# kdexd/probnmn-clevr

Hardware: AMD Instinct MI355X
Metric: CLEVR questions/sec (joint_training step) (higher is better)
Workload: dtype f32; 1 GPU; joint_training_ours.yml (NMN + seq2seq + REINFORCE), global batch 1024 = 1024 questions per GPU x 1 (BASELINE configs[3]), 14x14x1024 features, half of the batch with program supervision, fwd+bwd+[all-reduce]+clamp+Adam; global_batch=1024, per_gpu_batch=1024, parallelism=dp1

## Files before the change

### probnmn-clevr_amd/csrc/conv_stream.h

```cpp
#pragma once
#include <hip/hip_runtime.h>
#include <stdint.h>

#include <type_traits>

#include "../../include/probnmn_hip.h"
#include "global_ptr.h"

#ifdef PNMN_STREAM_CYCLES
#define PNMN_CYC() __builtin_readcyclecounter()
#else
#define PNMN_CYC() 0ull
#endif

namespace pnmn {
namespace stream {

constexpr int CB = 128;
constexpr int QC = 32;
constexpr int NTHREADS = 512;
constexpr int LOADER_WAVE = 4;
constexpr int NLOAD = 4;
constexpr int MTILES = 13;
constexpr int TAB_ROWS = 208;

using lchar = __attribute__((address_space(3))) char;

template <int H, int W, int TH>
struct Geom {
    static constexpr bool WHOLE = (TH == H);
    static constexpr int NB = H / TH;
    static constexpr int RP = (WHOLE ? H : TH + 2) * W;
    static constexpr int Z0 = (RP + 7) & ~7;
    static constexpr int SUB_PIECES = (Z0 + 15) / 16;
    static constexpr int PIECES = 2 * SUB_PIECES;
    static constexpr int SUB_BYTES = (Z0 + 8) * 64;
    static constexpr int SLOT_BYTES = 2 * SUB_BYTES;
    static constexpr int RING = WHOLE ? 6 : 4;
    static constexpr bool OVERLAP = (Z0 % 16) != 0;
    static constexpr int owner(int i) { return (OVERLAP && i == SUB_PIECES - 1) ? (SUB_PIECES - 2) % NLOAD : i % NLOAD; }
    static constexpr int owned(int lw) {
        int n = 0;
        for (int i = 0; i < SUB_PIECES; ++i) n += owner(i) == lw ? 1 : 0;
        return n;
    }
    static constexpr int TAB_OFF = RING * SLOT_BYTES;
    static constexpr int LDS_BYTES = TAB_OFF + 9 * TAB_ROWS * 2 + 128;
    static_assert(LDS_BYTES <= 160 * 1024, "ring + table must fit the CU's LDS");
    static_assert((Z0 + 7) * 64 + 16 < 65536 && SUB_BYTES < 65536, "table entries and the kb offset are 16 bits");
};

struct Launch {
    int n_seg;
    int wg_begin[3], split[3], unit0[3], n_units[3], per_xcd[3];
    int wgs_x;
    int total;
    int cin_chunks, ntaps, in_stride, out_stride, relu;
    unsigned long long* dbg;
};

__device__ __forceinline__ void lds_barrier() {
    asm volatile("s_waitcnt lgkmcnt(0)\n\ts_barrier" ::: "memory");
}

template <int H, int W, int TH>
__device__ __forceinline__ bool pass_rows(int band, int dil, int npass, int pass, int ntaps, int& rs, int& re, int& t0, int& t1) {
    if (Geom<H, W, TH>::WHOLE) {
        rs = 0, re = H, t0 = 0, t1 = ntaps;
        return true;
    }
    const int y0 = band * TH;
    if (npass == 1) {
        const int halo = (ntaps == 1) ? 0 : 1;
        rs = y0 - halo < 0 ? 0 : y0 - halo;
        re = y0 + TH + halo > H ? H : y0 + TH + halo;
        t0 = 0, t1 = ntaps;
        return true;
    }
    const int a = y0 + (pass - 1) * dil;
    rs = a < 0 ? 0 : (a > H ? H : a);
    re = a + TH < 0 ? 0 : (a + TH > H ? H : a + TH);
    t0 = 3 * pass, t1 = t0 + 3;
    return re > rs;
}

template <int H, int W, int TH>
struct Walker {
    using G = Geom<H, W, TH>;
    const pnmn_conv_item* items;
    int vid, total;
    int item, band, sub, split, cb;
    int dil, npass, slots;
    int chunk, pass, kq;
    int rs, re, t0, t1;

    __device__ __forceinline__ bool valid() const { return vid < total; }

    __device__ __forceinline__ bool decode(const Launch& L) {
        const int cout_blocks = L.total / L.wgs_x;
        const int s8 = vid >> 3;
        const int cbi = s8 % cout_blocks;
        const int x = (s8 / cout_blocks) * 8 + (vid & 7);
        int wb = L.wg_begin[0], sp = L.split[0], u0 = L.unit0[0], nu = L.n_units[0], per = L.per_xcd[0];
        if (L.n_seg > 1 && x >= L.wg_begin[1]) wb = L.wg_begin[1], sp = L.split[1], u0 = L.unit0[1], nu = L.n_units[1], per = L.per_xcd[1];
        if (L.n_seg > 2 && x >= L.wg_begin[2]) wb = L.wg_begin[2], sp = L.split[2], u0 = L.unit0[2], nu = L.n_units[2], per = L.per_xcd[2];
        const int local = x - wb;
        const int slot = local >> 3;
        const int j = slot / sp;
        const int unit = (local & 7) * per + j;
        if (unit >= nu || j >= per) return false;
        const int u = u0 + unit;
        item = u / G::NB, band = u % G::NB, sub = slot - j * sp, split = sp, cb = cbi;
        return true;
    }
    __device__ __forceinline__ void open_unit(const Launch& L) {
        while (vid < total && !decode(L)) vid += (int)gridDim.x;
        if (vid >= total) return;
        const pnmn_conv_item* it = items + item;
        dil = it->dilation;
        slots = it->gate ? 2 : 1;
        npass = (G::WHOLE || L.ntaps == 1 || dil == 1) ? 1 : 3;
        chunk = 0, pass = 0, kq = 0;
        while (!pass_rows<H, W, TH>(band, dil, npass, pass, L.ntaps, rs, re, t0, t1)) ++pass;
    }
    __device__ __forceinline__ void start(const Launch& L, const pnmn_conv_item* its) {
        items = its, vid = (int)blockIdx.x, total = L.total;
        open_unit(L);
    }
    __device__ __forceinline__ bool next_stage(const Launch& L) {
        if (++kq < 4) return true;
        kq = 0;
        while (++pass < npass)
            if (pass_rows<H, W, TH>(band, dil, npass, pass, L.ntaps, rs, re, t0, t1)) return true;
        if (++chunk >= L.cin_chunks) return false;
        pass = 0;
        while (!pass_rows<H, W, TH>(band, dil, npass, pass, L.ntaps, rs, re, t0, t1)) ++pass;
        return true;
    }
    __device__ __forceinline__ void next_unit(const Launch& L) {
        vid += (int)gridDim.x;
        open_unit(L);
    }
    __device__ __forceinline__ int cbase() const { return chunk * CB + kq * QC; }
};


template <int N>
__device__ __forceinline__ void wait_vm() {
    asm volatile("s_waitcnt vmcnt(%0)" ::"n"(N) : "memory");
}

template <int H, int W, int TH, int LW>
__device__ __forceinline__ void issue_rows(const float* src, int in_stride, int rs, int re, lchar* slot, int lane) {
    using G = Geom<H, W, TH>;
    const int nr = (re - rs) * W;
    using gchar = __attribute__((address_space(1))) char;
    const uint64_t src64 = (uint64_t)(uintptr_t)src + (uint64_t)rs * W * in_stride * 4;
    const uint64_t base64 = ((uint64_t)(uint32_t)__builtin_amdgcn_readfirstlane((int)(src64 >> 32)) << 32) |
                            (uint32_t)__builtin_amdgcn_readfirstlane((int)(uint32_t)src64);
    const gchar* base = (const gchar*)base64;
    const int s = lane & 3, lrow = lane >> 2;
    const int g = (((s & 1) ^ ((lane >> 4) & 1)) << 1) | (s >> 1);
    const uint32_t voff = (uint32_t)(lrow * in_stride + g * 4) * 4u;
    const int edge = (nr & 15) && nr < G::Z0 ? (nr < G::Z0 - 16 ? nr & ~15 : G::Z0 - 16) : -1;
    const uint32_t eoff = edge < 0 ? voff : (uint32_t)(((edge + lrow < nr ? edge + lrow : nr - 1) - edge) * in_stride + g * 4) * 4u;
#pragma unroll
    for (int i = 0; i < G::SUB_PIECES; ++i) {
        if (G::owner(i) != LW) continue;
        const int r0 = i * 16 < G::Z0 - 16 ? i * 16 : G::Z0 - 16;
        const uint32_t off = r0 == edge ? eoff : voff;
        const gchar* pb = base + (size_t)(r0 < nr ? r0 : 0) * in_stride * 4;
        __builtin_amdgcn_global_load_lds((const gfloat*)(pb + off), slot + r0 * 64, 16, 0, 0);
        __builtin_amdgcn_global_load_lds((const gfloat*)(pb + (off + 64u)), slot + G::SUB_BYTES + r0 * 64, 16, 0, 0);
    }
}

template <int H, int W, int TH, int LW>
__device__ __forceinline__ void fixup(char* lds, int slot_x, int slot_g, const float* mask, int rs, int re, bool gated, int lane) {
    using G = Geom<H, W, TH>;
    const int nr = (re - rs) * W;
    const gfloat* msrc = mask ? as_global(mask) + rs * W : nullptr;
    float mk[G::SUB_PIECES];
#pragma unroll
    for (int i = 0; i < G::SUB_PIECES; ++i) {
        if (G::owner(i) != LW) continue;
        const int row = i * 16 + (lane >> 2);
        mk[i] = msrc ? msrc[row < nr ? row : nr - 1] : 1.f;
    }
#pragma unroll
    for (int kb = 0; kb < 2; ++kb) {
        f32x4 v[G::SUB_PIECES], gt[G::SUB_PIECES];
#pragma unroll
        for (int i = 0; i < G::SUB_PIECES; ++i) {
            if (G::owner(i) != LW) continue;
            const int off = kb * G::SUB_BYTES + i * 1024 + lane * 16;
            v[i] = *reinterpret_cast<const f32x4*>(lds + slot_x + off);
            if (gated) gt[i] = *reinterpret_cast<const f32x4*>(lds + slot_g + off);
        }
#pragma unroll
        for (int i = 0; i < G::SUB_PIECES; ++i) {
            if (G::owner(i) != LW) continue;
            const int off = kb * G::SUB_BYTES + i * 1024 + lane * 16;
            f32x4 x = v[i] * mk[i];
            if (gated) {
                x.x = gt[i].x > 0.f ? x.x : 0.f;
                x.y = gt[i].y > 0.f ? x.y : 0.f;
                x.z = gt[i].z > 0.f ? x.z : 0.f;
                x.w = gt[i].w > 0.f ? x.w : 0.f;
            }
            if (i * 16 + (lane >> 2) < G::Z0) *reinterpret_cast<f32x4*>(lds + slot_x + off) = x;
        }
    }
}

template <int H, int W, int TH>
__device__ __forceinline__ void fill_table(char* lds, int band, int dil, int npass, int ntaps, int lane, int w, int nw) {
    using G = Geom<H, W, TH>;
    constexpr int HW = TH * W;
    uint16_t* tab = reinterpret_cast<uint16_t*>(lds + G::TAB_OFF);
    const int y0 = G::WHOLE ? 0 : band * TH;
    const int ntile = ntaps * MTILES;
    for (int t4 = 4 * w; t4 < ntile; t4 += 4 * nw) {
        const int tile = t4 + (lane >> 4);
        const int tap = tile / MTILES;
        const int m = tile - tap * MTILES;
        const int p = m * 16 + (lane & 15);
        int rs, re, t0, t1;
        const int pass = npass == 1 ? 0 : tap / 3;
        const bool rows_ok = tile < ntile && pass_rows<H, W, TH>(band, dil, npass, pass, ntaps, rs, re, t0, t1);
        int dy = 0, dx = 0;
        if (ntaps == 9) dy = (tap / 3 - 1) * dil, dx = (tap % 3 - 1) * dil;
        const int yy = y0 + p / W + dy, xx = p % W + dx;
        const bool ok = rows_ok && p < HW && yy >= rs && yy < re && (unsigned)xx < (unsigned)W;
        const int qv = rows_ok ? (yy - rs) * W + xx : p;
        const int row = ok ? qv : G::Z0 + (qv & 7);
        if (tile < ntile) tab[tap * TAB_ROWS + p] = (uint16_t)(row * 64 + ((row >> 2) & 1) * 16);
    }
}

template <int H, int W, int TH>
__device__ __forceinline__ void start_up(char* lds, const Walker<H, W, TH>& first, int ntaps, int wave, int lane) {
    using G = Geom<H, W, TH>;
    for (int t = wave * 64 + lane; t < G::RING * 64; t += NTHREADS) {
        const int sl = t >> 6, kb = (t >> 5) & 1;
        *reinterpret_cast<f32x4*>(lds + sl * G::SLOT_BYTES + kb * G::SUB_BYTES + G::Z0 * 64 + (t & 31) * 16) = f32x4{0.f, 0.f, 0.f, 0.f};
    }
    if (first.valid()) fill_table<H, W, TH>(lds, first.band, first.dil, first.npass, ntaps, lane, wave, NTHREADS / 64);
    lds_barrier();
}

template <int H, int W, int TH, int LW>
__device__ __forceinline__ void loader(const Launch& L, const pnmn_conv_item* items, char* lds, int lane) {
    using G = Geom<H, W, TH>;
    constexpr int NP2 = 2 * G::owned(LW);
    lchar* ring = (lchar*)lds;
    __builtin_amdgcn_s_setprio(3);
    Walker<H, W, TH> P, C;
    P.start(L, items);
    C = P;
    int issued = 0, freed = 0, cstart = 0;
    const pnmn_conv_item* pit = P.valid() ? items + P.item : nullptr;
    auto top_up = [&](int limit) {
        while (P.valid() && issued - freed + P.slots <= limit) {
            const float* src = (pit->in2 != nullptr && P.chunk > 0) ? pit->in2 + P.kq * QC : pit->in + P.cbase();
            issue_rows<H, W, TH, LW>(src, L.in_stride, P.rs, P.re, ring + (issued % G::RING) * G::SLOT_BYTES, lane);
            if (P.slots == 2) {
                issue_rows<H, W, TH, LW>(pit->gate + P.cbase(), L.in_stride, P.rs, P.re,
                                     ring + ((issued + 1) % G::RING) * G::SLOT_BYTES, lane);
            }
            issued += P.slots;
            if (!P.next_stage(L)) {
                P.next_unit(L);
                pit = P.valid() ? items + P.item : nullptr;
            }
        }
    };
    bool unit_end = false;
    unsigned long long lc[4] = {0, 0, 0, 0};
    unsigned long long lt = PNMN_CYC();
    auto lap = [&](int k) {
        const unsigned long long now = PNMN_CYC();
        lc[k] += now - lt;
        lt = now;
    };
    auto prepare = [&] {
        const pnmn_conv_item* cit = items + C.item;
        const int younger = issued - (cstart + C.slots);
        if (younger == 0) wait_vm<0>();
        else if (younger == 1) wait_vm<NP2>();
        else if (younger == 2) wait_vm<2 * NP2>();
        else wait_vm<3 * NP2>();
        lap(1);
        if (cit->mask != nullptr || C.slots == 2)
            fixup<H, W, TH, LW>(lds, (cstart % G::RING) * G::SLOT_BYTES, ((cstart + 1) % G::RING) * G::SLOT_BYTES, cit->mask, C.rs,
                            C.re, C.slots == 2, lane);
        lap(2);
    };
    top_up(P.valid() ? P.slots : 0);
    int tab_band = C.valid() ? C.band : -1, tab_dil = C.valid() ? C.dil : -1;
    start_up<H, W, TH>(lds, C, L.ntaps, LOADER_WAVE + LW, lane);
    lap(0);
    bool prepared = false;
    while (C.valid()) {
        if (!prepared) prepare();
        if (unit_end) {
            lds_barrier();
            unit_end = false;
            lap(3);
        }
        if (C.band != tab_band || C.dil != tab_dil) {
            fill_table<H, W, TH>(lds, C.band, C.dil, C.npass, L.ntaps, lane, LW, NLOAD);
            tab_band = C.band, tab_dil = C.dil;
        }
        lap(2);
        lds_barrier();
        lap(3);
        freed = cstart;
        cstart += C.slots;
        if (!C.next_stage(L)) {
            C.next_unit(L);
            unit_end = true;
        }
        prepared = C.valid() && issued >= cstart + C.slots;
        if (prepared) prepare();
        top_up(G::RING);
        lap(0);
    }
    if (unit_end) lds_barrier();
    if (L.dbg && lane == 0 && LW == 0) {
        unsigned long long* d = L.dbg + ((size_t)gridDim.x * 4 + blockIdx.x) * 8;
        d[0] = lc[0], d[1] = lc[1], d[2] = lc[2], d[3] = lc[3];
    }
}


__device__ __forceinline__ void mfma(f32x4& acc, float a, float b) {
    asm volatile("v_mfma_f32_16x16x4_f32 %0, %1, %2, %0" : "+v"(acc) : "v"(a), "v"(b));
}


template <int H, int W, int TH, int MTW>
__device__ __forceinline__ void epilogue(const pnmn_conv_item& it, const f32x4* acc, int mbase, int n0, int band, int out_stride,
                                         int relu, int lane, const f32x4 bias4) {
    constexpr int HW = TH * W;
    asm volatile("" : "+v"(lane));
    const int li = lane & 15, g = lane >> 4;
    const int p_img = Geom<H, W, TH>::WHOLE ? 0 : band * TH * W;
    auto act = [&](f32x4 v) {
        v += bias4;
        if (relu) {
            v.x = fmaxf(v.x, 0.f);
            v.y = fmaxf(v.y, 0.f);
            v.z = fmaxf(v.z, 0.f);
            v.w = fmaxf(v.w, 0.f);
        }
        return v;
    };
    float* const out0 = it.out + (size_t)p_img * out_stride + n0 + 4 * g;
    if (!(it.flags & (PNMN_CONV_ACCUMULATE | PNMN_CONV_MASKBWD | PNMN_CONV_DATTN))) {
#pragma unroll
        for (int j = 0; j < MTW; ++j) {
            const int p = (mbase + j) * 16 + li;
            if (p < HW) store4(as_global(out0 + (size_t)p * out_stride), act(acc[j]));
        }
        return;
    }
    if (it.flags & PNMN_CONV_DATTN) {
        const bool dattn = it.mb_attn != nullptr;
        f32x4 fv[MTW];
#pragma unroll
        for (int j = 0; j < MTW; ++j) {
            const int p = (mbase + j) * 16 + li;
            fv[j] = (dattn && p < HW) ? load4(as_global(it.mb_feats) + (size_t)(p_img + p) * CB + n0 + 4 * g) : f32x4{0.f, 0.f, 0.f, 0.f};
        }
#pragma unroll
        for (int j = 0; j < MTW; ++j) {
            const int p = (mbase + j) * 16 + li;
            if (p < HW) store4(as_global(out0 + (size_t)p * out_stride), act(acc[j]));
        }
        if (dattn) {
#pragma unroll
            for (int j = 0; j < MTW; ++j) {
                const int p = (mbase + j) * 16 + li;
                const f32x4 v = acc[j];
                float part = (p < HW) ? v.x * fv[j].x + v.y * fv[j].y + v.z * fv[j].z + v.w * fv[j].w : 0.f;
                part += __shfl_xor(part, 16);
                part += __shfl_xor(part, 32);
                if (p < HW && g == 0) unsafeAtomicAdd(it.mb_dattn + p_img + p, part);
            }
        }
        return;
    }
    if (it.flags & PNMN_CONV_MASKBWD) {
        const bool sole = it.flags & PNMN_CONV_MB_SOLE;
        const gfloat* attn = as_global(it.mb_attn);
        float am[MTW];
        f32x4 fv[MTW], dold[MTW];
#pragma unroll
        for (int j = 0; j < MTW; ++j) {
            const int p = (mbase + j) * 16 + li;
            const bool ok = p < HW;
            am[j] = (ok && attn) ? attn[p_img + p] : 1.f;
            fv[j] = (ok && attn) ? load4(as_global(it.mb_feats) + (size_t)(p_img + p) * CB + n0 + 4 * g) : f32x4{0.f, 0.f, 0.f, 0.f};
            dold[j] = (ok && sole) ? load4(as_global(it.mb_dfeats) + (size_t)(p_img + p) * CB + n0 + 4 * g) : f32x4{0.f, 0.f, 0.f, 0.f};
        }
#pragma unroll
        for (int j = 0; j < MTW; ++j) {
            const int p = (mbase + j) * 16 + li;
            const bool ok = p < HW;
            const f32x4 v = acc[j];
            float part = v.x * fv[j].x + v.y * fv[j].y + v.z * fv[j].z + v.w * fv[j].w;
            if (ok) {
                float* d = it.mb_dfeats + (size_t)(p_img + p) * CB + n0 + 4 * g;
                if (sole) {
                    store4(as_global(d), dold[j] + v * am[j]);
                } else {
                    unsafeAtomicAdd(d + 0, v.x * am[j]);
                    unsafeAtomicAdd(d + 1, v.y * am[j]);
                    unsafeAtomicAdd(d + 2, v.z * am[j]);
                    unsafeAtomicAdd(d + 3, v.w * am[j]);
                }
            }
            if (attn) {
                part += __shfl_xor(part, 16);
                part += __shfl_xor(part, 32);
                if (ok && g == 0) unsafeAtomicAdd(it.mb_dattn + p_img + p, part);
            }
        }
        return;
    }
    if (it.flags & PNMN_CONV_ATOMIC) {
#pragma unroll
        for (int j = 0; j < MTW; ++j) {
            const int p = (mbase + j) * 16 + li;
            if (p < HW) {
                const f32x4 v = act(acc[j]);
                float* d = out0 + (size_t)p * out_stride;
                unsafeAtomicAdd(d + 0, v.x);
                unsafeAtomicAdd(d + 1, v.y);
                unsafeAtomicAdd(d + 2, v.z);
                unsafeAtomicAdd(d + 3, v.w);
            }
        }
        return;
    }
    f32x4 old[MTW];
#pragma unroll
    for (int j = 0; j < MTW; ++j) {
        const int p = (mbase + j) * 16 + li;
        old[j] = p < HW ? load4(as_global(out0 + (size_t)p * out_stride)) : f32x4{0.f, 0.f, 0.f, 0.f};
    }
#pragma unroll
    for (int j = 0; j < MTW; ++j) {
        const int p = (mbase + j) * 16 + li;
        if (p < HW) store4(as_global(out0 + (size_t)p * out_stride), act(acc[j]) + old[j]);
    }
}

template <int H, int W, int TH, int MTW>
__device__ __forceinline__ void epilogue_plain_pair(const pnmn_conv_item& it, const f32x4* acc0, const f32x4* acc1, int mbase, int n0,
                                                    int band, int out_stride, int relu, int lane, const f32x4 bias0, const f32x4 bias1) {
    constexpr int HW = TH * W;
    asm volatile("" : "+v"(lane));
    const int li = lane & 15, g = lane >> 4;
    const int p_img = Geom<H, W, TH>::WHOLE ? 0 : band * TH * W;
    auto act = [&](f32x4 v, const f32x4 b) {
        v += b;
        if (relu) {
            v.x = fmaxf(v.x, 0.f);
            v.y = fmaxf(v.y, 0.f);
            v.z = fmaxf(v.z, 0.f);
            v.w = fmaxf(v.w, 0.f);
        }
        return v;
    };
    float* const out0 = it.out + (size_t)p_img * out_stride + n0 + 4 * g;
#pragma unroll
    for (int j = 0; j < MTW; ++j) {
        const int p = (mbase + j) * 16 + li;
        const f32x4 v0 = act(acc0[j], bias0), v1 = act(acc1[j], bias1);
        if (p < HW) {
            store4(as_global(out0 + (size_t)p * out_stride), v0);
            store4(as_global(out0 + (size_t)p * out_stride + 16), v1);
        }
        __builtin_amdgcn_sched_barrier(0);
    }
}

template <int H, int W, int TH, int SPLIT, int KIND>
__device__ __forceinline__ void run_unit(Walker<H, W, TH>& Wk, const Launch& L, char* lds, int& cstart, int wave, int lane,
                                         unsigned long long (&cyc)[4]) {
    using G = Geom<H, W, TH>;
    using std::integral_constant;
    const unsigned long long c_unit = PNMN_CYC();
    static_assert(SPLIT == 1 || SPLIT == 2 || SPLIT == 4 || SPLIT == 6 || SPLIT == 8 || SPLIT == 14 || SPLIT == 26,
                  "workgroups per 128-channel block");
    constexpr int NW = SPLIT == 1 ? 2 : 1;
    constexpr int MW = SPLIT <= 2 ? 1 : SPLIT / 2;
    constexpr int MTW = (MTILES + MW - 1) / MW;
    constexpr int MH = (MTW + 1) / 2;
    constexpr int WSETS = NW == 2 ? 2 : 3;
    constexpr uint32_t FULL = (1u << MTW) - 1u;
    const int li = lane & 15, g = lane >> 4;
    constexpr bool DEALT = (MW & (MW - 1)) != 0;
    const int gw = Wk.sub * 4 + wave;
    const int nt = DEALT ? 0 : wave % (4 / (DEALT ? 1 : MW));
    const int mbase = DEALT ? (gw % MW) * MTW : (wave / (4 / (DEALT ? 1 : MW))) * MTW;
    const pnmn_conv_item it = Wk.items[Wk.item];
    const int n0 = DEALT ? Wk.cb * CB + (gw / MW) * 16 : Wk.cb * CB + Wk.sub * (CB / SPLIT) + nt * 16 * NW;
    const int band = Wk.band;
    const int cin_total = L.cin_chunks * CB;
    const int slots = Wk.slots;

    f32x4 acc[NW][MTW];
#pragma unroll
    for (int n = 0; n < NW; ++n)
#pragma unroll
        for (int j = 0; j < MTW; ++j) acc[n][j] = f32x4{0.f, 0.f, 0.f, 0.f};

    constexpr int NTAPS = KIND == 2 ? 1 : 9;
    const gfloat* wrow = as_global(it.weight) + (size_t)(n0 + li) * NTAPS * cin_total + 4 * g;
    const size_t wtile = (size_t)16 * NTAPS * cin_total;
    const uint32_t gconst = (uint32_t)((g >> 1) * 16 | (g & 1) * 32);
    uint32_t tab_lane = (uint32_t)(G::TAB_OFF + (mbase * 16 + li) * 2);
    asm volatile("" : "+v"(tab_lane));
    const uint32_t exist = (mbase >= MTILES) ? 0u : (MTILES - mbase >= MTW ? FULL : ((1u << (MTILES - mbase)) - 1u));

    f32x4 bias4[NW];
#pragma unroll
    for (int n = 0; n < NW; ++n) {
        bias4[n] = f32x4{0.f, 0.f, 0.f, 0.f};
        if (it.bias) bias4[n] = load4(as_global(it.bias) + n0 + 16 * n + 4 * g);
    }
    f32x4 wq[WSETS][NW][2];
    auto wload = [&](f32x4 (&dst)[NW][2], const gfloat* p) {
#pragma unroll
        for (int n = 0; n < NW; ++n) {
            dst[n][0] = load4(p + n * wtile);
            dst[n][1] = load4(p + n * wtile + 16);
        }
    };
    {
        const gfloat* w0 = wrow + (size_t)Wk.t0 * cin_total + Wk.cbase();
        wload(wq[0], w0);
        if constexpr (WSETS == 3) wload(wq[1], KIND == 2 ? w0 + QC : w0 + cin_total);
    }

    uint32_t rb[MTW];
    f32x4 afrag[MTW];
    uint32_t slot_base = 0;
    using lf32x4 = __attribute__((address_space(3))) f32x4;
    const uint32_t lds0 = (uint32_t)(uintptr_t)(lchar*)lds;
    auto row_fetch = [&](int j, const char* tp) { rb[j] = *reinterpret_cast<const uint16_t*>(tp + j * 32); };
    auto row_apply = [&](int j) { rb[j] = (rb[j] ^ gconst) + slot_base; };
    auto frag_load = [&](int j, int kb) { afrag[j] = *reinterpret_cast<const lf32x4*>((uintptr_t)(rb[j] + kb * G::SUB_BYTES)); };

    auto half = [&](auto DO, auto LO, auto HI, const f32x4 (&bw)[NW][2], auto KB, auto NFILL, auto&& fill, auto&& reload) {
        constexpr int lo = decltype(LO)::value, hi = decltype(HI)::value, nfill = decltype(NFILL)::value, kb = decltype(KB)::value;
        constexpr int per = (hi - lo) * NW;
#pragma unroll
        for (int c = 0; c < 3; ++c)
#pragma unroll
            for (int j = lo; j < hi; ++j)
#pragma unroll
                for (int n = 0; n < NW; ++n) {
                    if (decltype(DO)::value) mfma(acc[n][j], bw[n][kb][c], afrag[j][c]);
                    if (c * per + (j - lo) * NW + n < nfill) fill(c * per + (j - lo) * NW + n);
                    __builtin_amdgcn_sched_barrier(0);
                }
#pragma unroll
        for (int j = lo; j < hi; ++j) {
#pragma unroll
            for (int n = 0; n < NW; ++n)
                if (decltype(DO)::value) mfma(acc[n][j], bw[n][kb][3], afrag[j][3]);
            reload(j);
            __builtin_amdgcn_sched_barrier(0);
        }
#pragma unroll
        for (int k = 3 * per; k < nfill; ++k) fill(k);
        __builtin_amdgcn_sched_barrier(0);
    };
    auto tap_body = [&](auto HALVES, auto SET, auto FAR, const char* tp, const gfloat* wfar) {
        constexpr int hv = decltype(HALVES)::value;
        constexpr int set = decltype(SET)::value, far = decltype(FAR)::value;
        using D0 = integral_constant<bool, hv == 0 || hv == 1>;
        using D1 = integral_constant<bool, hv == 0 || hv == 2>;
        using LO0 = integral_constant<int, 0>;
        using MID = integral_constant<int, MH>;
        using END = integral_constant<int, MTW>;
        using K0 = integral_constant<int, 0>;
        using K1 = integral_constant<int, 1>;
        auto fill0 = [&](int i) { wq[far][i >> 1][i & 1] = load4(wfar + (i >> 1) * wtile + (i & 1) * 16); };
        auto nofill = [&](int) {};
        auto reload1 = [&](int j) { frag_load(j, 1); };
        half(D0{}, LO0{}, MID{}, wq[set], K0{}, integral_constant<int, 2 * NW>{}, fill0, reload1);
        half(D1{}, MID{}, END{}, wq[set], K0{}, integral_constant<int, 0>{}, nofill, reload1);
        auto fill1 = [&](int i) {
            if (i < MTW) row_fetch(i, tp);
            else row_apply(i - MTW);
        };
        auto reload0 = [&](int j) { frag_load(j, 0); };
        constexpr int cap1 = 3 * MH * NW;
        static_assert(2 * MTW <= cap1 || NW == 1, "the first half must hold the row fillers");
        half(D0{}, LO0{}, MID{}, wq[set], K1{}, integral_constant<int, (2 * MTW < cap1 ? 2 * MTW : cap1)>{}, fill1, reload0);
        half(D1{}, MID{}, END{}, wq[set], K1{}, integral_constant<int, (2 * MTW > cap1 ? 2 * MTW - cap1 : 0)>{},
             [&](int i) { fill1(i + cap1); }, reload0);
    };
    using I0 = integral_constant<int, 0>;
    using I1 = integral_constant<int, 1>;
    using I2 = integral_constant<int, 2>;

    bool more = true;
    auto stage = [&](auto PAR) {
        constexpr int par = decltype(PAR)::value;
        const int t0 = Wk.t0, t1 = Wk.t1, cb0 = Wk.cbase();
        slot_base = lds0 + (uint32_t)((cstart % G::RING) * G::SLOT_BYTES);
        cstart += slots;
        more = Wk.next_stage(L);
        const gfloat* wnext_stage = more ? wrow + (size_t)Wk.t0 * cin_total + Wk.cbase() : wrow + (size_t)t0 * cin_total + cb0;
        auto far_ptr = [&](int tap, int d) -> const gfloat* {
            if (tap + d < t1) return wrow + (size_t)(tap + d) * cin_total + cb0;
            return more ? wnext_stage + (size_t)(tap + d - t1) * cin_total : wrow + (size_t)tap * cin_total + cb0;
        };
        auto next_row = [&](int tap) -> const char* { return lds + tab_lane + (tap + 1 < NTAPS ? tap + 1 : NTAPS - 1) * (TAB_ROWS * 2); };

        {
            const unsigned long long c0 = PNMN_CYC();
            lds_barrier();
            cyc[0] += PNMN_CYC() - c0;
        }
#pragma unroll
        for (int j = 0; j < MTW; ++j) row_fetch(j, lds + tab_lane + t0 * (TAB_ROWS * 2));
#pragma unroll
        for (int j = 0; j < MTW; ++j) row_apply(j);
#pragma unroll
        for (int j = 0; j < MTW; ++j) frag_load(j, 0);
        if constexpr (KIND == 2) {
            using SA = integral_constant<int, par>;
            using SB = integral_constant<int, (par + WSETS - 1) % WSETS>;
            const int ahead = cb0 + (WSETS - 1) * QC;
            tap_body(I0{}, SA{}, SB{}, next_row(0), wrow + (ahead < cin_total ? ahead : cb0));
        } else if constexpr (WSETS == 3) {
            if (KIND == 1) {
                tap_body(I2{}, I0{}, I2{}, next_row(0), far_ptr(0, 2));
                tap_body(I2{}, I1{}, I0{}, next_row(1), far_ptr(1, 2));
                tap_body(I2{}, I2{}, I1{}, next_row(2), far_ptr(2, 2));
                tap_body(I0{}, I0{}, I2{}, next_row(3), far_ptr(3, 2));
                tap_body(I0{}, I1{}, I0{}, next_row(4), far_ptr(4, 2));
                tap_body(I0{}, I2{}, I1{}, next_row(5), far_ptr(5, 2));
                tap_body(I1{}, I0{}, I2{}, next_row(6), far_ptr(6, 2));
                tap_body(I1{}, I1{}, I0{}, next_row(7), far_ptr(7, 2));
                tap_body(I1{}, I2{}, I1{}, next_row(8), far_ptr(8, 2));
            } else {
                for (int ta = t0; ta < t1; ta += 3) {
                    tap_body(I0{}, I0{}, I2{}, next_row(ta), far_ptr(ta, 2));
                    tap_body(I0{}, I1{}, I0{}, next_row(ta + 1), far_ptr(ta + 1, 2));
                    tap_body(I0{}, I2{}, I1{}, next_row(ta + 2), far_ptr(ta + 2, 2));
                }
            }
        } else {
            using SA = integral_constant<int, par>;
            using SB = integral_constant<int, par ^ 1>;
            if (KIND == 1) {
                tap_body(I2{}, SA{}, SB{}, next_row(0), far_ptr(0, 1));
                tap_body(I2{}, SB{}, SA{}, next_row(1), far_ptr(1, 1));
                tap_body(I2{}, SA{}, SB{}, next_row(2), far_ptr(2, 1));
                tap_body(I0{}, SB{}, SA{}, next_row(3), far_ptr(3, 1));
                tap_body(I0{}, SA{}, SB{}, next_row(4), far_ptr(4, 1));
                tap_body(I0{}, SB{}, SA{}, next_row(5), far_ptr(5, 1));
                tap_body(I1{}, SA{}, SB{}, next_row(6), far_ptr(6, 1));
                tap_body(I1{}, SB{}, SA{}, next_row(7), far_ptr(7, 1));
                tap_body(I1{}, SA{}, SB{}, next_row(8), far_ptr(8, 1));
            } else {
                int ta = t0;
                for (; ta + 1 < t1; ta += 2) {
                    tap_body(I0{}, SA{}, SB{}, next_row(ta), far_ptr(ta, 1));
                    tap_body(I0{}, SB{}, SA{}, next_row(ta + 1), far_ptr(ta + 1, 1));
                }
                tap_body(I0{}, SA{}, SB{}, next_row(ta), far_ptr(ta, 1));
            }
        }
    };
    while (more) {
        stage(I0{});
        if constexpr (WSETS == 2 || KIND == 2) {
            if (more) stage(I1{});
        }
        if constexpr (WSETS == 3 && KIND == 2) {
            if (more) stage(I2{});
        }
    }
    const unsigned long long c_u = PNMN_CYC();
    lds_barrier();
    const unsigned long long c_e = PNMN_CYC();
    if (exist != 0u) {
        if constexpr (NW == 2) {
            if (!(it.flags & (PNMN_CONV_ACCUMULATE | PNMN_CONV_MASKBWD | PNMN_CONV_DATTN))) {
                epilogue_plain_pair<H, W, TH, MTW>(it, acc[0], acc[1], mbase, n0, band, L.out_stride, L.relu, lane, bias4[0], bias4[NW - 1]);
            } else {
#pragma unroll
                for (int n = 0; n < NW; ++n)
                    epilogue<H, W, TH, MTW>(it, acc[n], mbase, n0 + 16 * n, band, L.out_stride, L.relu, lane, bias4[n]);
            }
        } else {
#pragma unroll
            for (int n = 0; n < NW; ++n)
                epilogue<H, W, TH, MTW>(it, acc[n], mbase, n0 + 16 * n, band, L.out_stride, L.relu, lane, bias4[n]);
        }
    }
    Wk.next_unit(L);
    const unsigned long long c_x = PNMN_CYC();
    cyc[0] += c_e - c_u;
    cyc[1] += c_x - c_e;
    cyc[2] += c_x - c_unit;
    cyc[3] += 1;
}

template <int H, int W, int TH, int TAPS>
__device__ __forceinline__ void conv_stream(const Launch& L, const pnmn_conv_item* items, char* lds) {
    static_assert(TAPS == 9 || TAPS == 1, "3x3 or 1x1");
    using G = Geom<H, W, TH>;
    const int tid = threadIdx.x;
    const int wave = __builtin_amdgcn_readfirstlane(tid >> 6);
    const int lane = tid & 63;
    if (wave >= LOADER_WAVE) {
        switch (wave - LOADER_WAVE) {
            case 0: loader<H, W, TH, 0>(L, items, lds, lane); break;
            case 1: loader<H, W, TH, 1>(L, items, lds, lane); break;
            case 2: loader<H, W, TH, 2>(L, items, lds, lane); break;
            default: loader<H, W, TH, 3>(L, items, lds, lane); break;
        }
        return;
    }
    Walker<H, W, TH> Wk;
    Wk.start(L, items);
    start_up<H, W, TH>(lds, Wk, L.ntaps, wave, lane);
    int cstart = 0;
    unsigned long long cyc[4] = {0, 0, 0, 0};
    const unsigned long long c_begin = PNMN_CYC();
    while (Wk.valid()) {
        if constexpr (TAPS == 1) {
            switch (Wk.split) {
                case 1: run_unit<H, W, TH, 1, 2>(Wk, L, lds, cstart, wave, lane, cyc); break;
                case 2: run_unit<H, W, TH, 2, 2>(Wk, L, lds, cstart, wave, lane, cyc); break;
                case 4: run_unit<H, W, TH, 4, 2>(Wk, L, lds, cstart, wave, lane, cyc); break;
                default: run_unit<H, W, TH, 8, 2>(Wk, L, lds, cstart, wave, lane, cyc); break;
            }
        } else if (G::WHOLE && Wk.dil == 8 && Wk.split <= 2) {
            if (Wk.split == 1) run_unit<H, W, TH, 1, 1>(Wk, L, lds, cstart, wave, lane, cyc);
            else run_unit<H, W, TH, 2, 1>(Wk, L, lds, cstart, wave, lane, cyc);
        } else {
            switch (Wk.split) {
                case 1: run_unit<H, W, TH, 1, 0>(Wk, L, lds, cstart, wave, lane, cyc); break;
                case 2: run_unit<H, W, TH, 2, 0>(Wk, L, lds, cstart, wave, lane, cyc); break;
                case 4: run_unit<H, W, TH, 4, 0>(Wk, L, lds, cstart, wave, lane, cyc); break;
                case 6: run_unit<H, W, TH, 6, 0>(Wk, L, lds, cstart, wave, lane, cyc); break;
                case 14: run_unit<H, W, TH, 14, 0>(Wk, L, lds, cstart, wave, lane, cyc); break;
                case 26: run_unit<H, W, TH, 26, 0>(Wk, L, lds, cstart, wave, lane, cyc); break;
                default: run_unit<H, W, TH, 8, 0>(Wk, L, lds, cstart, wave, lane, cyc); break;
            }
        }
    }
    if (L.dbg && lane == 0) {
        unsigned long long* d = L.dbg + ((size_t)blockIdx.x * 4 + wave) * 8;
        d[0] = cyc[0], d[1] = cyc[1], d[2] = cyc[2], d[3] = cyc[3], d[4] = PNMN_CYC() - c_begin;
    }
}

}
}
```

Before: 38520 questions/s.

## Use 4x4x1 MFMA for the partial last pixel tile in whole-image conv

```diff
diff --git a/probnmn-clevr_amd/csrc/conv_stream.h b/probnmn-clevr_amd/csrc/conv_stream.h
--- a/probnmn-clevr_amd/csrc/conv_stream.h
+++ b/probnmn-clevr_amd/csrc/conv_stream.h
@@ -23,6 +23,8 @@
 constexpr int NLOAD = 4;
 constexpr int MTILES = 13;
 constexpr int TAB_ROWS = 208;
+constexpr int TAIL_TILE = 12;
+constexpr int TAIL_P0 = 192;
 
 using lchar = __attribute__((address_space(3))) char;
 
@@ -224,7 +226,7 @@
         const int tile = t4 + (lane >> 4);
         const int tap = tile / MTILES;
         const int m = tile - tap * MTILES;
-        const int p = m * 16 + (lane & 15);
+        const int p = (G::WHOLE && m * 16 + (lane & 15) >= HW) ? TAIL_P0 + (lane & 3) : m * 16 + (lane & 15);
         int rs, re, t0, t1;
         const int pass = npass == 1 ? 0 : tap / 3;
         const bool rows_ok = tile < ntile && pass_rows<H, W, TH>(band, dil, npass, pass, ntaps, rs, re, t0, t1);
@@ -234,7 +236,7 @@
         const bool ok = rows_ok && p < HW && yy >= rs && yy < re && (unsigned)xx < (unsigned)W;
         const int qv = rows_ok ? (yy - rs) * W + xx : p;
         const int row = ok ? qv : G::Z0 + (qv & 7);
-        if (tile < ntile) tab[tap * TAB_ROWS + p] = (uint16_t)(row * 64 + ((row >> 2) & 1) * 16);
+        if (tile < ntile) tab[tap * TAB_ROWS + m * 16 + (lane & 15)] = (uint16_t)(row * 64 + ((row >> 2) & 1) * 16);
     }
 }
 
@@ -338,6 +340,23 @@
     asm volatile("v_mfma_f32_16x16x4_f32 %0, %1, %2, %0" : "+v"(acc) : "v"(a), "v"(b));
 }
 
+template <bool PAD>
+__device__ __forceinline__ void mfma_tail(f32x4& acc, float a, float b) {
+    if (PAD) asm volatile("v_mfma_f32_4x4x1_16b_f32 %0, %1, %2, %0\n\ts_nop 3" : "+v"(acc) : "v"(a), "v"(b));
+    else asm volatile("v_mfma_f32_4x4x1_16b_f32 %0, %1, %2, %0" : "+v"(acc) : "v"(a), "v"(b));
+}
+__device__ __forceinline__ void tail_gather(f32x4& acc, int lane) {
+    const int src = (lane & 48) | ((lane >> 4) << 2) | (lane & 3);
+    float v[4] = {acc.x, acc.y, acc.z, acc.w};
+#pragma unroll
+    for (int i = 0; i < 4; ++i) {
+        v[i] += __shfl_xor(v[i], 16);
+        v[i] += __shfl_xor(v[i], 32);
+        v[i] = __shfl(v[i], src);
+        if ((lane & 15) >= 4) v[i] = 0.f;
+    }
+    acc = f32x4{v[0], v[1], v[2], v[3]};
+}
 
 template <int H, int W, int TH, int MTW>
 __device__ __forceinline__ void epilogue(const pnmn_conv_item& it, const f32x4* acc, int mbase, int n0, int band, int out_stride,
@@ -487,9 +506,9 @@
     }
 }
 
-template <int H, int W, int TH, int SPLIT, int KIND>
-__device__ __forceinline__ void run_unit(Walker<H, W, TH>& Wk, const Launch& L, char* lds, int& cstart, int wave, int lane,
-                                         unsigned long long (&cyc)[4]) {
+template <int H, int W, int TH, int SPLIT, int KIND, bool TAIL>
+__device__ __forceinline__ void run_unit_body(Walker<H, W, TH>& Wk, const Launch& L, char* lds, int& cstart, int wave, int lane,
+                                              unsigned long long (&cyc)[4]) {
     using G = Geom<H, W, TH>;
     using std::integral_constant;
     const unsigned long long c_unit = PNMN_CYC();
@@ -499,6 +518,7 @@
     constexpr int MW = SPLIT <= 2 ? 1 : SPLIT / 2;
     constexpr int MTW = (MTILES + MW - 1) / MW;
     constexpr int MH = (MTW + 1) / 2;
+    constexpr int JT = TAIL ? TAIL_TILE % MTW : -1;
     constexpr int WSETS = NW == 2 ? 2 : 3;
     constexpr uint32_t FULL = (1u << MTW) - 1u;
     const int li = lane & 15, g = lane >> 4;
@@ -564,7 +584,10 @@
             for (int j = lo; j < hi; ++j)
 #pragma unroll
                 for (int n = 0; n < NW; ++n) {
-                    if (decltype(DO)::value) mfma(acc[n][j], bw[n][kb][c], afrag[j][c]);
+                    if (decltype(DO)::value) {
+                        if (j == JT) mfma_tail<MTW <= 2>(acc[n][j], bw[n][kb][c], afrag[j][c]);
+                        else mfma(acc[n][j], bw[n][kb][c], afrag[j][c]);
+                    }
                     if (c * per + (j - lo) * NW + n < nfill) fill(c * per + (j - lo) * NW + n);
                     __builtin_amdgcn_sched_barrier(0);
                 }
@@ -572,7 +595,10 @@
         for (int j = lo; j < hi; ++j) {
 #pragma unroll
             for (int n = 0; n < NW; ++n)
-                if (decltype(DO)::value) mfma(acc[n][j], bw[n][kb][3], afrag[j][3]);
+                if (decltype(DO)::value) {
+                    if (j == JT) mfma_tail<MTW <= 2>(acc[n][j], bw[n][kb][3], afrag[j][3]);
+                    else mfma(acc[n][j], bw[n][kb][3], afrag[j][3]);
+                }
             reload(j);
             __builtin_amdgcn_sched_barrier(0);
         }
@@ -693,6 +719,10 @@
     const unsigned long long c_u = PNMN_CYC();
     lds_barrier();
     const unsigned long long c_e = PNMN_CYC();
+    if constexpr (TAIL) {
+#pragma unroll
+        for (int n = 0; n < NW; ++n) tail_gather(acc[n][JT], lane);
+    }
     if (exist != 0u) {
         if constexpr (NW == 2) {
             if (!(it.flags & (PNMN_CONV_ACCUMULATE | PNMN_CONV_MASKBWD | PNMN_CONV_DATTN))) {
@@ -714,6 +744,22 @@
     cyc[1] += c_x - c_e;
     cyc[2] += c_x - c_unit;
     cyc[3] += 1;
+}
+
+template <int H, int W, int TH, int SPLIT, int KIND>
+__device__ __forceinline__ void run_unit(Walker<H, W, TH>& Wk, const Launch& L, char* lds, int& cstart, int wave, int lane,
+                                         unsigned long long (&cyc)[4]) {
+    if constexpr (!Geom<H, W, TH>::WHOLE) {
+        run_unit_body<H, W, TH, SPLIT, KIND, false>(Wk, L, lds, cstart, wave, lane, cyc);
+    } else if constexpr (SPLIT <= 2) {
+        run_unit_body<H, W, TH, SPLIT, KIND, true>(Wk, L, lds, cstart, wave, lane, cyc);
+    } else {
+        constexpr int MW = SPLIT / 2, MTW = (MTILES + MW - 1) / MW;
+        constexpr bool DEALT = (MW & (MW - 1)) != 0;
+        const int mbase = DEALT ? ((Wk.sub * 4 + wave) % MW) * MTW : (wave / (4 / (DEALT ? 1 : MW))) * MTW;
+        if (mbase <= TAIL_TILE && TAIL_TILE < mbase + MTW) run_unit_body<H, W, TH, SPLIT, KIND, true>(Wk, L, lds, cstart, wave, lane, cyc);
+        else run_unit_body<H, W, TH, SPLIT, KIND, false>(Wk, L, lds, cstart, wave, lane, cyc);
+    }
 }
 
 template <int H, int W, int TH, int TAPS>
```

New measurement: 38500 questions/s. About the same (-0.0%).
